# balbasty/torch-interpol

Measured on AMD Instinct MI355X. Metric: Mvox/s grid_pull & grid_push, 256^3 fp32 cubic/dct2, higher is better.
Workload: dtype f32

## Files before the change

### include/interpol_hip.h

```cpp
#ifndef INTERPOL_HIP_H
#define INTERPOL_HIP_H

#include <stdint.h>

#ifdef __cplusplus
extern "C" {
#endif

#define INTERPOL_ABI_VERSION 1

enum {
    INTERPOL_F32  = 0,
    INTERPOL_F64  = 1,
    INTERPOL_BF16 = 2,
    INTERPOL_F16  = 3
};

enum {
    INTERPOL_OK          =  0,
    INTERPOL_E_DIM       = -1,
    INTERPOL_E_ORDER     = -2,
    INTERPOL_E_BOUND     = -3,
    INTERPOL_E_DTYPE     = -4,
    INTERPOL_E_SHAPE     = -5,
    INTERPOL_E_NULL      = -6,
    INTERPOL_E_EXTRAP    = -7,
    INTERPOL_E_PREFILTER = -8,
    INTERPOL_E_SCRATCH   = -9,
    INTERPOL_E_STRIDE    = -10,
    INTERPOL_E_LAUNCH    = -11
};

typedef struct interpol_problem {
    int32_t abi_version;
    int32_t dim;
    int32_t dtype;
    int32_t grid_dtype;
    int32_t extrapolate;
    int32_t bound[3];
    int32_t order[3];
    int32_t flags;
    int64_t batch;
    int64_t channels;
    int64_t vol_shape[3];
    int64_t grid_shape[3];
    int64_t vol_stride[5];
    int64_t grid_stride[5];
    int64_t val_stride[7];
} interpol_problem;

#define INTERPOL_FLAG_NO_FASTPATH   1
#define INTERPOL_FLAG_ACCUMULATE    2
#define INTERPOL_FLAG_FORCE_TILED   4
#define INTERPOL_FLAG_SEPARABLE_GRID 8
#define INTERPOL_FLAG_DISPLACEMENT  16
#define INTERPOL_FLAG_WITH_COUNT    32
#define INTERPOL_FLAG_BINNED_SCATTER 64
#define INTERPOL_FLAG_AUTO_SCATTER  (1 << 24)
#define INTERPOL_FLAG_SMALL_TILES (1 << 25)
#define INTERPOL_FLAG_SERIAL_ITEMS (1 << 26)
#define INTERPOL_FLAG_GENERAL_KERNELS (1 << 27)
#define INTERPOL_FLAG_AFFINE_GRID   128

int64_t interpol_scatter_workspace(const interpol_problem *p, int32_t count_only);
int interpol_pull(const interpol_problem *p, const void *vol, const void *grid, void *val, void *stream);
int64_t interpol_pull_workspace(const interpol_problem *p);
int interpol_pull_ws(const interpol_problem *p, const void *vol, const void *grid, void *val, void *workspace, int64_t workspace_bytes, void *stream);
int interpol_grad_ws(const interpol_problem *p, const void *vol, const void *grid, void *val, void *workspace, int64_t workspace_bytes, void *stream);
int interpol_push(const interpol_problem *p, const void *val, const void *grid, void *vol,
                  void *scratch, int64_t scratch_bytes, void *stream);
int interpol_count(const interpol_problem *p, const void *grid, void *vol,
                   void *scratch, int64_t scratch_bytes, void *stream);
int interpol_grad(const interpol_problem *p, const void *vol, const void *grid, void *val, void *stream);
int interpol_pushgrad(const interpol_problem *p, const void *val, const void *grid, void *vol,
                      void *scratch, int64_t scratch_bytes, void *stream);
int interpol_hess(const interpol_problem *p, const void *vol, const void *grid, void *val, void *stream);

int interpol_pull_backward(const interpol_problem *p, const void *grad_out, const void *vol, const void *grid,
                           void *grad_vol, void *grad_grid, void *scratch, int64_t scratch_bytes, void *stream);
int interpol_push_backward(const interpol_problem *p, const void *grad_vol_out, const void *val, const void *grid,
                           void *grad_val, void *grad_grid, void *stream);
int interpol_count_backward(const interpol_problem *p, const void *grad_vol_out, const void *grid,
                            void *grad_grid, void *stream);
int interpol_push_backward_ws(const interpol_problem *p, const void *grad_vol_out, const void *val, const void *grid,
                              void *grad_val, void *grad_grid, void *workspace, int64_t workspace_bytes, void *stream);

int64_t interpol_affine_backward_workspace(const interpol_problem *p);
int interpol_pull_backward_affine(const interpol_problem *p, const void *grad_out, const void *vol,
                                  const void *mat, void *grad_mat,
                                  void *workspace, int64_t workspace_bytes, void *stream);
int interpol_push_backward_affine(const interpol_problem *p, const void *grad_vol_out,
                                  const void *val , const void *mat, void *grad_mat,
                                  void *workspace, int64_t workspace_bytes, void *stream);

int interpol_compose(const interpol_problem *p, const void *left, const void *right, void *out, void *stream);
int interpol_compose_backward_right(const interpol_problem *p, const void *grad_out, const void *left, const void *right,
                                    void *grad_right, void *stream);

int64_t interpol_push_bricks_workspace(const interpol_problem *p);
int interpol_push_bricks(const interpol_problem *p, const void *val, const void *grid, void *vol,
                         void *workspace, int64_t workspace_bytes, void *stream);

int interpol_pull_labels(const interpol_problem *p, const void *vol, const void *grid, void *val, void *stream);

int interpol_resample_1d(int32_t dtype, int32_t lin_dtype, int32_t order, int32_t bound, int32_t extrapolate, int32_t mode,
                         int32_t adjoint, int64_t outer, int64_t n_samples, int64_t n_lattice, int64_t inner,
                         const void *src, const void *lin, void *dst, void *stream);
int32_t interpol_resample_1d_gathers(int32_t dtype, int64_t n_samples, int64_t inner);

int interpol_spline_filter(void *data, int32_t dtype, int64_t outer, int64_t n, int64_t inner,
                           int32_t bound, int32_t order, void *stream);
int interpol_spline_filter_to(const void *src, void *data, int32_t dtype, int64_t outer, int64_t n, int64_t inner,
                              int32_t bound, int32_t order, void *stream);

// ... 21 lines not shown
```

### torch-interpol_amd/csrc/push_owner.hip

```cpp
#include "sorted_util.hpp"

namespace ip {
namespace owner {

using namespace sorted;

constexpr int BR = 16;
constexpr int OFF = 160;
constexpr int BOX = BR + 3;
constexpr int PZ = BOX;
constexpr int PLANE = BOX * PZ;
constexpr int BOXSLOTS = BOX * PLANE;
constexpr int NCELL = BR * BR * BR;
constexpr int CAPD = 128;
constexpr int CAPX = 512;
constexpr int NT = 512;
constexpr int NS = TS * TS * TS;
constexpr int NT1 = 512, VPT1 = NS / NT1;
constexpr int LB = 6, NBIN = LB * LB * LB;
constexpr int HDR_SHELL = 34;
constexpr int KMIX = 13;
template <int K> constexpr int KSV = K == KMIX ? 3 : K;
template <int K> __device__ __forceinline__ int kd(const KParams &p, int d) { return K == KMIX ? p.order[d] : K; }
#ifdef IP_OWNER_MIX_TU
#define IP_KS KSV<K>
#define IP_KD(d) kd<K>(p, d)
#define IP_WX(i) own_weight_x<K>(p, tx, i)
#define IP_MU magic_units_p<K>(p)
#else
#define IP_KS K
#define IP_KD(d) K
#define IP_WX(i) weight_x<K>(tx, i)
#define IP_MU magic_units<K>()
#endif

constexpr int NLO = OFF / BR, NHI = (OFF + 3 + BR - 1) / BR;
struct BrickGrid {
    int nb[3];
    int lo[3], top[3], nin[3], split[3];
    int per_item;
    int item;
    int capd;
};
__host__ __device__ __forceinline__ bool folds(int bound, int n) { return (bound == B_REPLICATE || bound == B_DCT1 || bound == B_DCT2) && n >= 2 * BR; }
static BrickGrid brick_grid(const KParams &k)
{
    BrickGrid g;
    const bool mixed = k.order[0] != k.order[1] || k.order[0] != k.order[2];
    for (int d = 0; d < 3; ++d) {
        const int K = mixed ? 3 : k.order[d], n = k.vol_n[d];
        const bool f = folds(k.bound[d], n);
        g.lo[d] = f ? -(BOX - 1) / 2 : 0;
        g.top[d] = f ? n - (BOX + 1) / 2 + BR : (n - K > 0 ? n - K : 0);
        g.nin[d] = (g.top[d] - g.lo[d] + BR - 1) / BR;
        if (f) {
            const int c = g.top[d] - g.lo[d] - BR * (g.nin[d] - 1);
            if (c < K) { g.top[d] -= c; g.nin[d] -= 1; }
        }
        g.split[d] = f ? g.nin[d] / 2 : (g.nin[d] > 0 ? g.nin[d] - 1 : 0);
        g.nb[d] = NLO + g.nin[d] + NHI;
    }
    g.per_item = g.nb[0] * g.nb[1] * g.nb[2];
    g.item = g.per_item; g.capd = 128;
    return g;
}
__host__ __device__ __forceinline__ int brick_and_cell(int ft, int lo, int top, int nin, int split)
{
    if (ft < lo) return ((ft - lo + OFF) >> 4) | (((ft - lo + OFF) & (BR - 1)) << 16);
    if (ft >= top) return (NLO + nin + ((ft - top) >> 4)) | (((ft - top) & (BR - 1)) << 16);
    const int u = ft - lo, v = top - 1 - ft;
    const bool hi = u >= BR * split && (v >> 4) < nin - 1 - split;
    return hi ? (NLO + nin - 1 - (v >> 4)) | ((BR - 1 - (v & (BR - 1))) << 16) : (NLO + (u >> 4)) | ((u & (BR - 1)) << 16);
}
__host__ __device__ __forceinline__ int brick_origin(int bk, int lo, int top, int nin, int split)
{
    if (bk < NLO) return lo + bk * BR - OFF;
    if (bk >= NLO + nin) return top + (bk - NLO - nin) * BR;
    const int j = bk - NLO;
    return j <= split ? lo + j * BR : top - (nin - j) * BR;
}

struct BinSmem {
    int lo[3], total;
    int cnt[NBIN];
    int base[NBIN];
    int bmx[2];
    int orph, pad_;
    int gbk[NBIN];
};

template <typename T>
__device__ __forceinline__ float src_value(const KParams &p, const T *__restrict__ val, int64_t b, int64_t o, int ch, float m)
{
    if (val == nullptr || ch >= p.C) return m;
    return m * Cvt<float, T>::ld(val[b * p.val_sb + ch * p.val_sc + o]);
}

template <typename T, int K, int GM>
__device__ __forceinline__ void scatter_direct(const KParams &p, const T *__restrict__ val, const float *__restrict__ grid, float *__restrict__ vol,
                                            int64_t b, TileGeom g, int tid, unsigned mask, int nch)
{
    Lattice L;
#pragma unroll
    for (int d = 0; d < 3; ++d) { L.bound[d] = p.bound[d]; L.n[d] = p.vol_n[d]; L.ss[d] = p.vol_ss[d] / 4; L.k[d] = kd<K>(p, d); }
    L.lin = 0;
#pragma unroll 1
    for (int v = 0; v < VPT1; ++v) {
        if (!((mask >> v) & 1)) continue;
        int ox, oy, oz; float x[3];
        sample_pos(g, tid + NT1 * v, ox, oy, oz);
        load_xyz<GM>(p, grid, b, g, ox, oy, oz, x);
        const int64_t o = ((int64_t)ox * g.gy + oy) * g.gz + oz;
        const float m = inb_mask(p, x);
        if (KSV<K> == 1 && p.mode == MODE_ISO0) {
            const long long pk0 = wrap_outofline(L.bound[0], __float2int_rn(rintf(x[0])), L.n[0]);
            const long long pk1 = wrap_outofline(L.bound[1], __float2int_rn(rintf(x[1])), L.n[1]);
            const long long pk2 = wrap_outofline(L.bound[2], __float2int_rn(rintf(x[2])), L.n[2]);
            const float sgn = (float)((int)(pk0 >> 32) * (int)(pk1 >> 32) * (int)(pk2 >> 32));
            float *q = vol + b * p.vol_sb + (int)(pk0 & 0xffffffffll) * L.ss[0] + (int)(pk1 & 0xffffffffll) * L.ss[1] + (int)(pk2 & 0xffffffffll) * L.ss[2];
#pragma unroll 1
            for (int ch = 0; ch < nch; ++ch)
                __hip_atomic_fetch_add(q + (int64_t)ch * p.vol_sc, src_value<T>(p, val, b, o, ch, m) * sgn, __ATOMIC_RELAXED, __HIP_MEMORY_SCOPE_AGENT);
            continue;
        }
        int ii[3]; float tt[3];
#pragma unroll
        for (int d = 0; d < 3; ++d) split(kd<K>(p, d), x[d], ii[d], tt[d]);
#pragma unroll 1
        for (int ch = 0; ch < nch; ++ch)
            tiled::scatter_one_thread(L, vol + b * p.vol_sb + ch * p.vol_sc, src_value<T>(p, val, b, o, ch, m), ii[0], ii[1], ii[2], tt[0], tt[1], tt[2]);
    }
}

template <typename T, int K, int GM>
__device__ __forceinline__ void gather_direct(const KParams &p, const T *__restrict__ img, const float *__restrict__ grid, T *__restrict__ out,
                                              int64_t b, TileGeom g, int tid, unsigned mask)
{
    Lattice L;
#pragma unroll
    for (int d = 0; d < 3; ++d) { L.bound[d] = p.bound[d]; L.n[d] = p.vol_n[d]; L.ss[d] = p.vol_ss[d] / (int)sizeof(T); L.k[d] = kd<K>(p, d); }
    L.lin = 0;
#pragma unroll 1
    for (int v = 0; v < VPT1; ++v) {
        if (!((mask >> v) & 1)) continue;
        int ox, oy, oz; float x[3];
        sample_pos(g, tid + NT1 * v, ox, oy, oz);
        load_xyz<GM>(p, grid, b, g, ox, oy, oz, x);
        const int64_t o = ((int64_t)ox * g.gy + oy) * g.gz + oz;
        const float m = inb_mask(p, x);
        int ii[3]; float tt[3];
#pragma unroll
        for (int d = 0; d < 3; ++d) split(kd<K>(p, d), x[d], ii[d], tt[d]);
#pragma unroll 1
        for (int ch = 0; ch < p.C; ++ch)
            out[b * p.val_sb + ch * p.val_sc + o] = Cvt<float, T>::st(m * tiled::gather_one_thread<T>(L, img + b * p.vol_sb + ch * p.vol_sc, ii[0], ii[1], ii[2], tt[0], tt[1], tt[2], -1));
    }
}

template <typename T, int K, int GM>
__device__ __forceinline__ void gradc_direct(const KParams &p, const T *__restrict__ img, const T *__restrict__ gout, const float *__restrict__ grid,
                                             float *__restrict__ ggrid, int64_t b, TileGeom g, int tid, unsigned mask)
{
    Lattice L;
#pragma unroll
    for (int d = 0; d < 3; ++d) { L.bound[d] = p.bound[d]; L.n[d] = p.vol_n[d]; L.ss[d] = p.vol_ss[d] / (int)sizeof(T); L.k[d] = kd<K>(p, d); }
    L.lin = 0;
#pragma unroll 1
    for (int v = 0; v < VPT1; ++v) {
        if (!((mask >> v) & 1)) continue;
        int ox, oy, oz; float x[3];
        sample_pos(g, tid + NT1 * v, ox, oy, oz);
        load_xyz<GM>(p, grid, b, g, ox, oy, oz, x);
        const int64_t o = ((int64_t)ox * g.gy + oy) * g.gz + oz;
        const float m = inb_mask(p, x);
        int ii[3]; float tt[3];
#pragma unroll
        for (int d = 0; d < 3; ++d) split(kd<K>(p, d), x[d], ii[d], tt[d]);
        float a[3] = { 0.f, 0.f, 0.f };
#pragma unroll 1
        for (int ch = 0; ch < p.C; ++ch) {
            const float gv = gout ? Cvt<float, T>::ld(gout[b * p.val_sb + ch * p.val_sc + o]) : 1.f;
#pragma unroll 1
            for (int d = 0; d < 3; ++d)
                a[d] = __builtin_fmaf(gv, tiled::gather_one_thread<T>(L, img + b * p.vol_sb + ch * p.vol_sc, ii[0], ii[1], ii[2], tt[0], tt[1], tt[2], d), a[d]);
        }
        float *dst = ggrid + (b * p.N + o) * 3;
        dst[0] = a[0] * m; dst[1] = a[1] * m; dst[2] = a[2] * m;
    }
}

template <typename T, int K, int GM>
__device__ __forceinline__ void grad_direct(const KParams &p, const T *__restrict__ img, const float *__restrict__ grid, T *__restrict__ out,
                                            int64_t b, TileGeom g, int tid, unsigned mask)
{
    Lattice L;
#pragma unroll
    for (int d = 0; d < 3; ++d) { L.bound[d] = p.bound[d]; L.n[d] = p.vol_n[d]; L.ss[d] = p.vol_ss[d] / (int)sizeof(T); L.k[d] = kd<K>(p, d); }
    L.lin = 0;
#pragma unroll 1
    for (int v = 0; v < VPT1; ++v) {
        if (!((mask >> v) & 1)) continue;
        int ox, oy, oz; float x[3];
        sample_pos(g, tid + NT1 * v, ox, oy, oz);
        load_xyz<GM>(p, grid, b, g, ox, oy, oz, x);
        const int64_t o = ((int64_t)ox * g.gy + oy) * g.gz + oz;
        const float m = inb_mask(p, x);
        int ii[3]; float tt[3];
#pragma unroll
        for (int d = 0; d < 3; ++d) split(kd<K>(p, d), x[d], ii[d], tt[d]);
#pragma unroll 1
        for (int ch = 0; ch < p.C; ++ch)
#pragma unroll 1
            for (int d = 0; d < 3; ++d)
                out[b * p.val_sb + ch * p.val_sc + 3 * o + d] =
                    Cvt<float, T>::st(m * tiled::gather_one_thread<T>(L, img + b * p.vol_sb + ch * p.vol_sc, ii[0], ii[1], ii[2], tt[0], tt[1], tt[2], d));
    }
}

template <typename T, int K, int GM, int IDX = 0>
__global__ __launch_bounds__(NT1, 4) void own_bin(KParams p, BrickGrid bg, const T *__restrict__ val, const float *__restrict__ grid,
                                               float *__restrict__ vol, int *__restrict__ ndesc, uint2 *__restrict__ desc,
                                               float4 *__restrict__ rec, float *__restrict__ vals, unsigned short *__restrict__ meta,
                                               int *__restrict__ bmax, int64_t nrec,
                                               int gx, int gy, int gz, int nty, int ntz, int ntiles, const int *__restrict__ gate,
                                               const T *__restrict__ aux, const int *__restrict__ all, int blk0)
{
    const int blk = (int)blockIdx.x + blk0;
    if (IDX) { const bool every = all && *all == 1; if (gate ? (gate[blk] == 0 && !every) : (all && !every)) return; }
    else if (gate && *gate != 1) return;
    extern __shared__ __attribute__((aligned(16))) unsigned char smem_raw[];
    BinSmem &sm = *reinterpret_cast<BinSmem *>(smem_raw);
    const int tid = threadIdx.x;
    const int64_t b = blk / ntiles;
    const TileGeom g = tile_geom(blk % ntiles, gx, gy, gz, nty, ntz);
    const int nch = (IDX || val == nullptr) ? 1 : p.C + p.cc;
    for (int i = tid; i < NBIN; i += NT1) { sm.cnt[i] = 0; sm.gbk[i] = -1; }
    if (tid < 2) sm.bmx[tid] = 0;
    if (tid == 2) sm.orph = 0;
    if (tid < 3) sm.lo[tid] = 0x7fffffff;
    float c[VPT1][3], v0[VPT1], v1[VPT1];
    unsigned valid = 0;
    prof_mark(-1);
    const bool has0 = !IDX && val != nullptr && p.C > 0, has1 = !IDX && val != nullptr && p.C > 1;
    const T *vp0 = has0 ? val + b * p.val_sb : reinterpret_cast<const T *>(grid);
    const T *vp1 = has1 ? val + b * p.val_sb + p.val_sc : reinterpret_cast<const T *>(grid);
#pragma unroll
    for (int v = 0; v < VPT1; ++v) {
        int ox, oy, oz;
        sample_pos(g, tid + NT1 * v, ox, oy, oz);
        if (ox < gx && oy < gy && oz < gz) valid |= 1u << v;
        ox = ox < gx ? ox : gx - 1; oy = oy < gy ? oy : gy - 1; oz = oz < gz ? oz : gz - 1;
        load_xyz<GM>(p, grid, b, g, ox, oy, oz, c[v]);
        const int64_t o = ((int64_t)ox * gy + oy) * gz + oz;
        if (IDX) { v0[v] = __int_as_float((int)o); v1[v] = 0.f; continue; }
        v0[v] = Cvt<float, T>::ld(vp0[has0 ? o : 0]);
        v1[v] = Cvt<float, T>::ld(vp1[has1 ? o : 0]);
    }
    unsigned inbits = 0;
#pragma unroll
    for (int v = 0; v < VPT1 && !IDX; ++v) {
        const float m = inb_mask(p, c[v]);
        v0[v] = has0 ? v0[v] * m : m; v1[v] = has1 ? v1[v] * m : m;
        if (KSV<K> == 1 && m != 0.f) inbits |= 1u << v;
    }
    if (KSV<K> == 1 && !IDX && p.mode == MODE_ISO0) {
#pragma unroll
        for (int v = 0; v < VPT1; ++v) { c[v][0] = rintf(c[v][0]); c[v][1] = rintf(c[v][1]); c[v][2] = rintf(c[v][2]); }
    }
    int bx[VPT1][3];
    unsigned ok = 0;
    int mn[3] = { 0x7fffffff, 0x7fffffff, 0x7fffffff };
#pragma unroll
    for (int v = 0; v < VPT1; ++v) {
        bool in = (valid >> v) & 1;
#pragma unroll
        for (int d = 0; d < 3; ++d) {
            const float fl = floorf(c[v][d] - 0.5f * (float)(kd<K>(p, d) - 1));
            in = in && fl >= (float)(bg.lo[d] - OFF) && fl < (float)(bg.top[d] + NHI * BR);
            bx[v][d] = in ? brick_and_cell(__float2int_rz(fl), bg.lo[d], bg.top[d], bg.nin[d], bg.split[d]) : 0;
        }
        if (in) {
            ok |= 1u << v;
#pragma unroll
            for (int d = 0; d < 3; ++d) mn[d] = (bx[v][d] & 0xffff) < mn[d] ? (bx[v][d] & 0xffff) : mn[d];
        }
    }
    __syncthreads();
    prof_mark(0);
#pragma unroll
    for (int d = 0; d < 3; ++d) {
        const int a = wave_min(mn[d]);
        if ((tid & 63) == 0) atomicMin(&sm.lo[d], a);
    }
    __syncthreads();
    const int lo[3] = { sm.lo[0], sm.lo[1], sm.lo[2] };
    int lbin[VPT1];
    unsigned local = 0;
#pragma unroll
    for (int v = 0; v < VPT1; ++v) {
        const int r0 = (bx[v][0] & 0xffff) - lo[0], r1 = (bx[v][1] & 0xffff) - lo[1], r2 = (bx[v][2] & 0xffff) - lo[2];
        const bool l = ((ok >> v) & 1) && (unsigned)r0 < (unsigned)LB && (unsigned)r1 < (unsigned)LB && (unsigned)r2 < (unsigned)LB;
        lbin[v] = l ? ((r0 * LB + r1) * LB + r2) | ((bx[v][0] >> 16) << 16 | (bx[v][1] >> 16) << 12 | (bx[v][2] >> 16) << 8) : 0;
        if (l) { local |= 1u << v; lbin[v] |= atomicAdd(&sm.cnt[lbin[v] & 255], 1) << 20; }
    }
    __syncthreads();
    prof_mark(1);
    const int64_t tilebase = (int64_t)blk * NS;
    constexpr int PER = (NBIN + 63) / 64;
    int slot[PER];
    if (tid < 64) {
        int cn[PER], s = 0;
#pragma unroll
        for (int i = 0; i < PER; ++i) { const int e = tid * PER + i; cn[i] = e < NBIN ? sm.cnt[e] : 0; s += cn[i]; }
        int incl = s;
#pragma unroll
        for (int o = 1; o < 64; o <<= 1) { const int t = __shfl_up(incl, o); if (tid >= o) incl += t; }
        int run = incl - s;
        if (tid == 63) sm.total = incl;
#pragma unroll
        for (int i = 0; i < PER; ++i) {
            const int e = tid * PER + i;
            const int r0 = e / (LB * LB), r1 = (e / LB) % LB, r2 = e % LB;
            const int bk = (int)b * bg.item + ((lo[0] + r0) * bg.nb[1] + (lo[1] + r1)) * bg.nb[2] + (lo[2] + r2);
            slot[i] = 0;
            if (e < NBIN) sm.base[e] = run;
            if (e < NBIN && cn[i] > 0) slot[i] = atomicAdd(&ndesc[bk], 1);
            run += cn[i];
        }
    }
    __syncthreads();
    prof_mark(2);
    int pos[VPT1];
#pragma unroll
    for (int v = 0; v < VPT1; ++v)
        pos[v] = ((local >> v) & 1) ? (sm.base[lbin[v] & 255] + (int)((unsigned)lbin[v] >> 20)) | (((lbin[v] >> 8) & 0xfff) << 16) : -1;
    const bool two = nch > 1;
    int amx0 = 0, amx1 = 0;
#pragma unroll
    for (int v = 0; v < VPT1; ++v) {
        if (pos[v] < 0) continue;
        const int64_t at = tilebase + (pos[v] & 0xffff);
        rec[at] = make_float4(c[v][0], c[v][1], c[v][2], v0[v]);
        if (IDX) continue;
        meta[at] = (unsigned short)(pos[v] >> 16);
        const int a0 = __float_as_int(__builtin_fabsf(v0[v]));
        amx0 = a0 > amx0 ? a0 : amx0;
        if (two) {
            vals[at] = v1[v];
            const int a1 = __float_as_int(__builtin_fabsf(v1[v]));
            amx1 = a1 > amx1 ? a1 : amx1;
        }
    }
    for (int ch = 2; ch < nch && !IDX; ++ch) {
#pragma unroll
        for (int v = 0; v < VPT1; ++v) {
            if (pos[v] < 0) continue;
            int ox, oy, oz;
            sample_pos(g, tid + NT1 * v, ox, oy, oz);
            vals[(int64_t)(ch - 1) * nrec + tilebase + (pos[v] & 0xffff)] = src_value<T>(p, val, b, ((int64_t)ox * gy + oy) * gz + oz, ch, KSV<K> == 1 ? (float)((inbits >> v) & 1u) : inb_mask(p, c[v]));
        }
    }
    if (tid < 64) {
#pragma unroll
        for (int i = 0; i < PER; ++i) {
            const int e = tid * PER + i;
            const int cn = e < NBIN ? sm.cnt[e] : 0;
            if (cn <= 0) continue;
            const int r0 = e / (LB * LB), r1 = (e / LB) % LB, r2 = e % LB;
            const int bk = (int)b * bg.item + ((lo[0] + r0) * bg.nb[1] + (lo[1] + r1)) * bg.nb[2] + (lo[2] + r2);
            if (slot[i] < bg.capd) {
                desc[(int64_t)bk * bg.capd + slot[i]] = make_uint2((unsigned)(tilebase + sm.base[e]), (unsigned)cn);
                sm.gbk[e] = bk;
                const int bc[3] = { lo[0] + r0, lo[1] + r1, lo[2] + r2 };
                bool shell = false;
#pragma unroll
                for (int d = 0; d < 3; ++d) shell = shell || bc[d] < NLO + (p.bound[d] == B_DST1 ? 1 : 0) || bc[d] >= NLO + bg.nin[d];
                if (!IDX && shell) ndesc[HDR_SHELL - 64] = 1;
                if (IDX && slot[i] == 0) bmax[1 + atomicAdd(&bmax[0], 1)] = bk;
            } else { sm.cnt[e] = -1; sm.orph = 1; }
        }
    }
    if (!IDX) {
        amx0 = wave_max(amx0); amx1 = wave_max(amx1);
        if ((tid & 63) == 0) { if (amx0) atomicMax(&sm.bmx[0], amx0); if (amx1) atomicMax(&sm.bmx[1], amx1); }
    }
    __syncthreads();
    for (int e = tid; e < NBIN && !IDX; e += NT1) {
        const int bk = sm.gbk[e];
        if (bk < 0) continue;
        if (sm.bmx[0]) atomicMax(&bmax[2 * (int64_t)bk], sm.bmx[0]);
        if (sm.bmx[1]) atomicMax(&bmax[2 * (int64_t)bk + 1], sm.bmx[1]);
    }
    unsigned direct = valid & ~local;
    if (sm.orph) {
#pragma unroll
        for (int v = 0; v < VPT1; ++v)
            if (((local >> v) & 1) && sm.cnt[lbin[v] & 255] < 0) direct |= 1u << v;
    }
    if (IDX == 3) { if (direct) grad_direct<T, K, GM>(p, val, grid, reinterpret_cast<T *>(vol), b, g, tid, direct); return; }
    if (IDX == 2) { if (direct) gradc_direct<T, K, GM>(p, val, aux, grid, vol, b, g, tid, direct); return; }
    if (IDX) { if (direct) gather_direct<T, K, GM>(p, val, grid, reinterpret_cast<T *>(vol), b, g, tid, direct); return; }
    if (direct) scatter_direct<T, K, GM>(p, val, grid, vol, b, g, tid, direct, nch);
}

constexpr int VPT = 12;
constexpr int NPIECE = VPT * (NT / 64);
constexpr int BATCH = NPIECE * 64;
constexpr int NCLS = 16;
constexpr int NHW = NT / NCLS;
constexpr unsigned PMASK = 0x1ffffffu;
static_assert(NPIECE <= 128, "a queue entry is piece << 6 | lane in 16 bits");

struct AccSmem {
    int   taboff[3][BOX + 1];
    float tabsgn[3][BOX + 1];
    unsigned ppref[CAPX];
    unsigned start[CAPX];
    uint2 piece[NPIECE];
    int   cmax[2];
    int   dmax, n, npieces;
    int   rlo[3], rhi[3];
    int   qcnt[NCLS];
    int   qsur[NCLS + 1], qhol[NCLS + 1];
    int   qeff[NCLS], qcap;
    union alignas(16) {
        struct {
            unsigned cells[NCELL / 2];
            unsigned short queue[BATCH];
        };
        unsigned nreg[BOX * BOX * (BOX + 1) / 2];
    };
    unsigned long long box[BOXSLOTS];
};
constexpr int NZ = BOX + 1;
static_assert(sizeof(AccSmem) <= 80 * 1024, "two workgroups per CU");
static_assert(sizeof(unsigned) * (BOX * BOX * NZ / 2) <= sizeof(unsigned) * (NCELL / 2) + sizeof(unsigned short) * BATCH, "the stencil counts fit in cells + queue");

constexpr float MAGIC = 12582912.f;
constexpr unsigned MAGIC_ODD = 301u;
template <int K> __device__ __forceinline__ float magic_units() { return K == 3 ? 4194304.f * 0.999f * 3.375f : (K == 2 ? 4194304.f * 0.999f * (64.f / 27.f) : 4194304.f * 0.999f); }
template <int K> __device__ __forceinline__ float magic_cbmax() { return 2147483648.f * 0.99f / magic_units<K>(); }
template <int K> __device__ __forceinline__ float magic_units_p(const KParams &p)
{
    if (K != KMIX) return magic_units<K>();
    float u = 4194304.f * 0.999f;
#pragma unroll
    for (int d = 0; d < 3; ++d) u *= p.order[d] == 3 ? 1.5f : (p.order[d] == 2 ? 4.f / 3.f : 1.f);
    return u;
}

// ... 1137 lines not shown
        if (cnt[2] == NS) { atomicAdd(&hdr->nbox, boxvol); atomicAdd(&hdr->nfull, 1); atomicAdd(&hdr->ncorner, cornervol); }
        __threadfence();
        if (atomicAdd(&hdr->done, 1) == (int)gridDim.x - 1) {
            const int ns = atomicAdd(&hdr->nslow, 0), nf = atomicAdd(&hdr->nfar, 0), nn = atomicAdd(&hdr->nvalid, 0);
            const int nb = atomicAdd(&hdr->nbox, 0), nt = atomicAdd(&hdr->nfull, 0), nc = atomicAdd(&hdr->ncorner, 0);
            const bool rough = nch > 1 && (int64_t)nb > (int64_t)BOXVOL * nt && (int64_t)nb * 10 > (int64_t)nc * 16;
            const bool dense = (int64_t)nc <= (int64_t)DENSEVOL * nt;
            if (nch == -2) hdr->gate = ((int64_t)ns * 1000 > (int64_t)nn * PULLOUT && (int64_t)nf * 64 <= nn) ? 1 : 0;
            else if (nch < 0) hdr->gate = (((int64_t)ns * 250 > nn || dense) && (int64_t)nf * 64 <= nn) ? 1 : 0;
            else hdr->gate = (((int64_t)ns * 250 > nn || rough) && (int64_t)nf * 64 <= nn) ? 1 : 0;
        }
    }
}

struct Workspace {
    int *flags;
    ProbeHdr *hdr; int *ndesc; int *bmax; uint2 *desc; float4 *rec; float *vals; unsigned short *meta;
    int64_t nrec; int nbricks;
};
static int64_t align256(int64_t x) { return (x + 255) & ~(int64_t)255; }

static int64_t layout(const KParams &k, int B, int ntiles, int nch, void *base, Workspace *w, int64_t nflags = 0, bool shared = false)
{
    const BrickGrid bg = brick_grid(k);
    const int64_t nbricks = (int64_t)bg.per_item * (shared ? 1 : B);
    const int64_t nrec = (int64_t)ntiles * NS * B;
    int64_t o = 0;
    unsigned char *p = (unsigned char *)base;
    const int64_t o_hdr = o; o += 256;
    const int64_t o_nd = o; o += nbricks * 4;
    const int64_t o_bm = o; o += nbricks * 8;
    const int64_t o_fl = o; o += nflags * 4; o = align256(o);
    const int64_t o_desc = o; o += align256(nbricks * (shared ? CAPX : CAPD) * 8);
    const int64_t o_rec = o; o += align256(nrec * 16);
    const int64_t o_val = o; o += align256(nrec * 4 * (nch > 1 ? nch - 1 : 0));
    const int64_t o_meta = o; o += align256(nrec * 2);
    if (w) {
        w->hdr = (ProbeHdr *)(p + o_hdr); w->ndesc = (int *)(p + o_nd); w->desc = (uint2 *)(p + o_desc);
        w->rec = (float4 *)(p + o_rec); w->vals = (float *)(p + o_val); w->meta = (unsigned short *)(p + o_meta);
        w->bmax = (int *)(p + o_bm); w->flags = (int *)(p + o_fl);
        w->nrec = nrec; w->nbricks = (int)nbricks;
    }
    return o;
}

static int tile_count(const interpol_problem *p)
{
    int64_t n = 1;
    for (int d = 0; d < 3; ++d) n *= (p->grid_shape[d] + TS - 1) / TS;
    return n > 0x7fffffff ? 0 : (int)n;
}

int mix_launch_bin(int dtype, int idx, const KParams &k, const BrickGrid &bg, const Workspace &w, const void *val, const void *grid, void *vol,
                   const int *gate, const void *aux, const int *all, int gx, int gy, int gz, int ntiles, int b0, int nb, hipStream_t st);
int mix_launch_acc(const KParams &k, const BrickGrid &bg, const Workspace &w, void *vol, int nch, int color, int b0, int nb, const int *gate,
                   int *ctr, unsigned nblocks, hipStream_t st);
int mix_launch_gather(int grad, const KParams &k, const BrickGrid &bg, const Workspace &w, const void *vol, void *val, const int *gate,
                      const void *gout, unsigned nblocks, hipStream_t st);

#ifdef IP_OWNER_MIX_TU
int mix_launch_bin(int dtype, int idx, const KParams &k, const BrickGrid &bg, const Workspace &w, const void *val, const void *grid, void *vol,
                   const int *gate, const void *aux, const int *all, int gx, int gy, int gz, int ntiles, int b0, int nb, hipStream_t st)
{
    const int nty = (gy + TS - 1) / TS, ntz = (gz + TS - 1) / TS;
    const dim3 tgrid((unsigned)(ntiles * nb));
#define IP_MIX_BIN(T, IDX)                                                                                              \
    {                                                                                                                   \
        const int attr = big_lds<own_bin<T, KMIX, 0, IDX>>(sizeof(BinSmem));                                            \
        if (attr) return attr;                                                                                          \
        hipLaunchKernelGGL((own_bin<T, KMIX, 0, IDX>), tgrid, dim3(NT1), sizeof(BinSmem), st, k, bg, (const T *)val, (const float *)grid, \
                           (float *)vol, w.ndesc, w.desc, w.rec, w.vals, w.meta, w.bmax, w.nrec, gx, gy, gz, nty, ntz, ntiles, gate, (const T *)aux, all, ntiles * b0); \
    }
    if (idx == 0) { if (dtype == INTERPOL_F32) IP_MIX_BIN(float, 0) else if (dtype == INTERPOL_BF16) IP_MIX_BIN(bf16_t, 0) else if (dtype == INTERPOL_F16) IP_MIX_BIN(f16_t, 0) else return INTERPOL_E_DTYPE; }
    else if (idx == 1) IP_MIX_BIN(float, 1) else if (idx == 2) IP_MIX_BIN(float, 2) else IP_MIX_BIN(float, 3)
#undef IP_MIX_BIN
    const hipError_t e = hipGetLastError();
    return e == hipSuccess ? 0 : (int)e;
}
int mix_launch_acc(const KParams &k, const BrickGrid &bg, const Workspace &w, void *vol, int nch, int color, int b0, int nb, const int *gate,
                   int *ctr, unsigned nblocks, hipStream_t st)
{
    const int attr = big_lds<own_accumulate<KMIX>>(sizeof(AccSmem));
    if (attr) return attr;
    hipLaunchKernelGGL((own_accumulate<KMIX>), dim3(nblocks), dim3(NT), sizeof(AccSmem), st, k, bg, (const int *)w.ndesc,
                       (const uint2 *)w.desc, (const float4 *)w.rec, (const float *)w.vals, (const unsigned short *)w.meta,
                       (const int *)w.bmax, w.nrec, (float *)vol, nch, color, nb, gate, ctr, b0, (const int *)w.hdr + HDR_SHELL);
    const hipError_t e = hipGetLastError();
    return e == hipSuccess ? 0 : (int)e;
}
int mix_launch_gather(int grad, const KParams &k, const BrickGrid &bg, const Workspace &w, const void *vol, void *val, const int *gate,
                      const void *gout, unsigned nblocks, hipStream_t st)
{
#define IP_MIX_GAT(GR)                                                                                                  \
    {                                                                                                                   \
        const int attr = big_lds<own_gather<KMIX, GR>>(sizeof(GatSmem));                                                \
        if (attr) return attr;                                                                                          \
        hipLaunchKernelGGL((own_gather<KMIX, GR>), dim3(nblocks), dim3(NT), sizeof(GatSmem), st, k, bg, (const int *)w.ndesc, (const uint2 *)w.desc, \
                           (const float4 *)w.rec, (const int *)w.bmax, (int *)w.hdr + 40, (const float *)vol, (float *)val, gate, (const float *)gout); \
    }
    if (grad == 1) IP_MIX_GAT(1) else if (grad == 2) IP_MIX_GAT(2) else IP_MIX_GAT(0)
#undef IP_MIX_GAT
    const hipError_t e = hipGetLastError();
    return e == hipSuccess ? 0 : (int)e;
}
#endif

}

#ifndef IP_OWNER_MIX_TU

static bool shared_target(const interpol_problem *p) { return p->vol_stride[0] == 0 && p->batch > 1; }
static bool mixed_orders(const KParams &k) { return k.order[0] != k.order[1] || k.order[0] != k.order[2]; }
static bool owner_eligible(const interpol_problem *p, const KParams &k, bool scatter = false)
{
    const bool shared = scatter && shared_target(p);
    if (p->dim != 3 || p->batch > 4096) return false;
    if (!(p->flags & (INTERPOL_FLAG_BINNED_SCATTER | INTERPOL_FLAG_AUTO_SCATTER))) return false;
    if (k.order[0] != k.order[1] || k.order[0] != k.order[2]) {
        for (int d = 0; d < 3; ++d) if (k.order[d] < 1 || k.order[d] > 3) return false;
        if (k.sep != 0) return false;
    } else if (k.order[0] < (scatter ? 1 : 2) || k.order[0] > 3) return false;
    int64_t n = 1, nv = 1, nb = shared ? 1 : p->batch;
    for (int d = 0; d < 3; ++d) {
        n *= p->grid_shape[d]; nv *= p->vol_shape[d];
        nb *= owner::NLO + owner::NHI + (p->vol_shape[d] + 15 + owner::BR - 1) / owner::BR;
        if (p->grid_shape[d] > 0x7fffffff / 4) return false;
    }
    const int64_t nt = owner::tile_count(p);
    if (n < 4096 || nt == 0 || nt * owner::NS * p->batch > 0x7fffffffll || nb > 0x7fffffffll / (shared ? owner::CAPX : owner::CAPD)) return false;
    if ((uint64_t)n * 12ull > 0xffffffffull) return false;
    return (shared ? 8 * n * p->batch : 4 * n) >= nv;
}

int linear_pull_probe(const interpol_problem *p, const KParams &k, const void *grid, void *workspace, hipStream_t st, const int **gate_out, int thr16);
constexpr int NEAREST_THR16 = 24;
static bool nearest_scatter(const KParams &k) { return k.dim == 3 && k.mode == MODE_ISO0 && k.order[0] == 0 && k.order[1] == 0 && k.order[2] == 0; }
static KParams nearest_as_trilinear(const KParams &k)
{
    KParams q = k;
    if (nearest_scatter(k)) { q.order[0] = 1; q.order[1] = 1; q.order[2] = 1; }
    return q;
}

int64_t owner_workspace_bytes(const interpol_problem *p, const KParams &k_in, bool count_only)
{
    const KParams k = nearest_as_trilinear(k_in);
    if (!owner_eligible(p, k, true)) return 0;
    const int nch = count_only ? 1 : k.C + (k.cc ? 1 : 0);
    return owner::layout(k, (int)p->batch, owner::tile_count(p), nch, nullptr, nullptr, 0, shared_target(p));
}

namespace owner {
template <typename T, int IDX = 0>
static int launch_bin(const interpol_problem *p, const KParams &k, const BrickGrid &bg, const Workspace &w, const void *val, const void *grid,
                      void *vol, const int *gate, hipStream_t st, const void *aux = nullptr, const int *all = nullptr,
                      int b0 = 0, int nb = -1)
{
    if (nb < 0) nb = (int)p->batch;
    const int gx = (int)p->grid_shape[0], gy = (int)p->grid_shape[1], gz = (int)p->grid_shape[2];
    const int nty = (gy + TS - 1) / TS, ntz = (gz + TS - 1) / TS;
    const int ntiles = tile_count(p);
    const dim3 tgrid((unsigned)(ntiles * nb));
    if (k.order[0] != k.order[1] || k.order[0] != k.order[2])
        return mix_launch_bin(std::is_same<T, float>::value ? INTERPOL_F32 : (std::is_same<T, bf16_t>::value ? INTERPOL_BF16 : INTERPOL_F16), IDX, k, bg, w,
                              val, grid, vol, gate, aux, all, gx, gy, gz, ntiles, b0, nb, st);
#define IP_OWN_BIN(KK, GM)                                                                                              \
    {                                                                                                                   \
        const int attr = big_lds<own_bin<T, KK, GM, IDX>>(sizeof(BinSmem));                                               \
        if (attr) return attr;                                                                                          \
        hipLaunchKernelGGL((own_bin<T, KK, GM, IDX>), tgrid, dim3(NT1), sizeof(BinSmem), st, k, bg, (const T *)val, (const float *)grid, \
                           (float *)vol, w.ndesc, w.desc, w.rec, w.vals, w.meta, w.bmax, w.nrec, gx, gy, gz, nty, ntz, ntiles, gate, (const T *)aux, all, ntiles * b0); \
    }
#define IP_OWN_BY_GM(KK)                                                                                                \
    { if (k.sep == 0) IP_OWN_BIN(KK, 0) else if (k.sep == 1) IP_OWN_BIN(KK, 1) else if (k.sep == 2) IP_OWN_BIN(KK, 2) else IP_OWN_BIN(KK, 3) }
    if (k.order[0] == 3) IP_OWN_BY_GM(3) else if (k.order[0] == 2) IP_OWN_BY_GM(2) else IP_OWN_BY_GM(1)
#undef IP_OWN_BY_GM
#undef IP_OWN_BIN
    return 0;
}
}

static int chain_counter(int chain, int color)
{
    static const int base[CHAIN_SIDE + 1] = { 16, 8 };
    return color < 8 ? base[chain] + color : 24;
}

int try_owner_push(const interpol_problem *p, const KParams &k_in, const void *val, const void *grid, void *vol,
                   void *workspace, int64_t workspace_bytes, hipStream_t st, const int **gate_out, PendingZero *zf)
{
    using namespace owner;
    const bool nearest = nearest_scatter(k_in);
    const KParams k = nearest_as_trilinear(k_in);
    if (!workspace || !owner_eligible(p, k, true)) return 0;
    const bool count_only = val == nullptr;
    const int nch = count_only ? 1 : k.C + (k.cc ? 1 : 0);
    const int dtype = count_only ? INTERPOL_F32 : p->dtype;
    if (dtype != INTERPOL_F32 && dtype != INTERPOL_BF16 && dtype != INTERPOL_F16) return 0;
    Workspace w;
    if (((uintptr_t)workspace & 255u) != 0) return 0;
    const bool shared = shared_target(p);
    if (layout(k, (int)p->batch, tile_count(p), nch, workspace, &w, 0, shared) > workspace_bytes) return 0;
    BrickGrid bg = brick_grid(k);
    if (shared) { bg.item = 0; bg.capd = CAPX; }
    const bool gated = !(p->flags & INTERPOL_FLAG_BINNED_SCATTER);
    if (nearest && gated && k.sep != 0 && k.sep != 2) return 0;
    const int B = (int)p->batch;
    ChainSet *cs = nullptr;
    if (!shared && B >= 2 && !(p->flags & INTERPOL_FLAG_SERIAL_ITEMS)) {
        hipStreamCaptureStatus cap = hipStreamCaptureStatusNone;
        if (hipStreamIsCapturing(st, &cap) != hipSuccess) { (void)hipGetLastError(); cap = hipStreamCaptureStatusActive; }
        if (cap == hipStreamCaptureStatusNone) cs = chains_acquire();
    }
    bool zero_pending = zf && zf->pending;
    const size_t slice = (size_t)k.vol_sb * 4;
    if (zero_pending && !(cs && zf->ptr == vol && slice * (size_t)B == zf->bytes)) {
        const hipError_t ez = zero_async(zf->ptr, zf->bytes, st);
        if (ez != hipSuccess) { chains_release(cs); return (int)ez; }
        zf->pending = zero_pending = false;
    }
    hipLaunchKernelGGL(own_zero, dim3((unsigned)((64 + 3ll * w.nbricks + 1023) / 1024)), dim3(1024), 0, st, (int *)w.hdr, 64 + 3 * w.nbricks);
    hipError_t e = hipGetLastError();
    if (e != hipSuccess) { chains_release(cs); return (int)e; }
    const int *gate = nullptr;
    if (gated && nearest) {
        const int rp = linear_pull_probe(p, k, grid, w.hdr, st, &gate, NEAREST_THR16);
        if (rp) { chains_release(cs); return rp; }
    } else if (gated) {
        const int gx = (int)p->grid_shape[0], gy = (int)p->grid_shape[1], gz = (int)p->grid_shape[2];
        const int nty = (gy + TS - 1) / TS, ntz = (gz + TS - 1) / TS, ntiles = tile_count(p);
        const long long total = (long long)ntiles * B;
        const dim3 pgrid((unsigned)(total < NPROBE ? total : NPROBE));
#define IP_OWN_PROBE(KK, GM) hipLaunchKernelGGL((own_probe<KK, GM>), pgrid, dim3(NT1), 0, st, k, bg, (const float *)grid, w.hdr, gx, gy, gz, nty, ntz, ntiles, B, nch);
#define IP_OWN_PROBE_GM(KK) { if (k.sep == 0) IP_OWN_PROBE(KK, 0) else if (k.sep == 1) IP_OWN_PROBE(KK, 1) else if (k.sep == 2) IP_OWN_PROBE(KK, 2) else IP_OWN_PROBE(KK, 3) }
        if (k.order[0] == 3 || mixed_orders(k)) IP_OWN_PROBE_GM(3) else if (k.order[0] == 2) IP_OWN_PROBE_GM(2) else IP_OWN_PROBE_GM(1)
#undef IP_OWN_PROBE_GM
#undef IP_OWN_PROBE
        gate = &w.hdr->gate;
    }
    const int nchain = B < CHAIN_SIDE + 1 ? B : CHAIN_SIDE + 1;
    if (cs) {
        bool ok = hipEventRecord(cs->fork, st) == hipSuccess;
        for (int i = 0; i + 1 < nchain && ok; ++i) ok = hipStreamWaitEvent(cs->side[i], cs->fork, 0) == hipSuccess;
        if (!ok) { (void)hipGetLastError(); chains_release(cs); cs = nullptr; }
    }
    if (zero_pending && !cs) {
        const hipError_t ez = zero_async(zf->ptr, zf->bytes, st);
        if (ez != hipSuccess) return (int)ez;
        zf->pending = zero_pending = false;
    }
    const long long want = 2ll * cu_count();
    const bool general = (p->flags & INTERPOL_FLAG_GENERAL_KERNELS) != 0;
    auto enqueue = [&](hipStream_t s, int chain, int b0, int nb) -> int {
        if (zero_pending) {
            const hipError_t ez = zero_async((char *)vol + (size_t)b0 * slice, (size_t)nb * slice, s);
            if (ez != hipSuccess) return (int)ez;
        }
        const int nbin = shared ? B : nb;
        int rc;
        switch (dtype) {
        case INTERPOL_F32: rc = launch_bin<float>(p, k, bg, w, val, grid, vol, gate, s, nullptr, nullptr, b0, nbin); break;
        case INTERPOL_BF16: rc = launch_bin<bf16_t>(p, k, bg, w, val, grid, vol, gate, s, nullptr, nullptr, b0, nbin); break;
        default: rc = launch_bin<f16_t>(p, k, bg, w, val, grid, vol, gate, s, nullptr, nullptr, b0, nbin); break;
        }
        if (rc) return rc;
        for (int color = 0; color < 9; ++color) {
            long long nwork = nb;
            for (int d = 0; d < 3; ++d) nwork *= color_count(color, d, bg);
            if (nwork <= 0) continue;
            const dim3 agrid((unsigned)(nwork < want ? nwork : want));
            int *ctr = (int *)w.hdr + chain_counter(chain, color);
#define IP_OWN_ACC_SH(KK, SH)                                                                                           \
            {                                                                                                           \
                const int attr = big_lds<own_accumulate<KK, false, SH>>(sizeof(AccSmem));                               \
                if (attr) return attr;                                                                                  \
                hipLaunchKernelGGL((own_accumulate<KK, false, SH>), agrid, dim3(NT), sizeof(AccSmem), s, k, bg, (const int *)w.ndesc, \
                                   (const uint2 *)w.desc, (const float4 *)w.rec, (const float *)w.vals, (const unsigned short *)w.meta,  \
                                   (const int *)w.bmax, w.nrec, (float *)vol, nch, color, nb, gate, ctr, b0,           \
                                   (const int *)w.hdr + HDR_SHELL);                                                     \
            }
#define IP_OWN_ACC(KK) { if (color < 8 && !general) IP_OWN_ACC_SH(KK, false) else IP_OWN_ACC_SH(KK, true) }
            if (mixed_orders(k)) { const int rm = mix_launch_acc(k, bg, w, vol, nch, color, b0, nb, gate, ctr, agrid.x, s); if (rm) return rm; }
            else if (k.order[0] == 3) IP_OWN_ACC(3) else if (k.order[0] == 2) IP_OWN_ACC(2)
            else if (nearest) {
                const int attr = big_lds<own_accumulate<1, true>>(sizeof(AccSmem));
                if (attr) return attr;
                hipLaunchKernelGGL((own_accumulate<1, true>), agrid, dim3(NT), sizeof(AccSmem), s, k, bg, (const int *)w.ndesc,
                                   (const uint2 *)w.desc, (const float4 *)w.rec, (const float *)w.vals, (const unsigned short *)w.meta,
                                   (const int *)w.bmax, w.nrec, (float *)vol, nch, color, nb, gate, ctr, b0, (const int *)w.hdr + HDR_SHELL);
            }
            else IP_OWN_ACC(1)
#undef IP_OWN_ACC
#undef IP_OWN_ACC_SH
        }
        const hipError_t el = hipGetLastError();
        return el == hipSuccess ? 0 : (int)el;
    };
    int rc = 0;
    if (!cs) rc = enqueue(st, 0, 0, shared ? 1 : B);
    else {
        for (int c = 1; c <= nchain && rc == 0; ++c) {
            const int ch = c % nchain, b0 = (int)((long long)ch * B / nchain), b1 = (int)((long long)(ch + 1) * B / nchain);
            rc = enqueue(ch ? cs->side[ch - 1] : st, ch, b0, b1 - b0);
        }
        if (zero_pending && rc == 0) zf->pending = false;
        for (int i = 0; i + 1 < nchain; ++i) {
            if (hipEventRecord(cs->join[i], cs->side[i]) == hipSuccess && hipStreamWaitEvent(st, cs->join[i], 0) == hipSuccess) continue;
            (void)hipGetLastError();
            const hipError_t es = hipStreamSynchronize(cs->side[i]);
            if (es != hipSuccess && rc == 0) rc = (int)es;
        }
        chains_release(cs);
    }
    if (rc) return rc;
    if (gate_out) *gate_out = gate;
    return gated ? 2 : 1;
// ... 171 lines not shown
```

### torch-interpol_amd/interpol/_hip.py

```python
import ctypes
import threading
import os

import torch

from .sepgrid import SeparableGrid, AffineGrid, LazyGrid

_PKG_ROOT = os.path.dirname(os.path.dirname(os.path.abspath(__file__)))
LIB_PATH = os.environ.get("INTERPOL_HIP_LIB") or os.path.join(_PKG_ROOT, "lib", "libinterpol_hip.so")

ABI_VERSION = 1
F32, F64, BF16, F16 = 0, 1, 2, 3
FLAG_NO_FASTPATH = 1
FLAG_ACCUMULATE = 2
FLAG_FORCE_TILED = 4
FLAG_SEPARABLE_GRID = 8
FLAG_DISPLACEMENT = 16
FLAG_WITH_COUNT = 32
FLAG_BINNED_SCATTER = 64
FLAG_AUTO_SCATTER = 1 << 24
_ROUTED_2D = (torch.float32, torch.bfloat16, torch.float16)
FLAG_SMALL_TILES = 1 << 25
FLAG_SERIAL_ITEMS = 1 << 26
FLAG_GENERAL_KERNELS = 1 << 27
_POISON_SCRATCH = os.environ.get("INTERPOL_POISON_SCRATCH", "0") not in ("", "0")
_WS_NOCACHE = os.environ.get("INTERPOL_WS_NOCACHE", "0") not in ("", "0")
FLAG_AFFINE_GRID = 128

def _empty(*size, **kw):
    return torch.empty(*size, **kw)


def _scratch(t):
    if _POISON_SCRATCH and t is not None:
        t.view(torch.uint8).fill_(0xff)
    return t


_DTYPE_CODE = {torch.float32: F32, torch.float64: F64, torch.bfloat16: BF16, torch.float16: F16}

SYMBOLS = (
    "interpol_pull", "interpol_push", "interpol_count", "interpol_grad", "interpol_pushgrad",
    "interpol_hess", "interpol_pull_backward", "interpol_push_backward", "interpol_count_backward",
    "interpol_spline_filter", "interpol_spline_filter_to", "interpol_resample_1d", "interpol_resample_1d_gathers", "interpol_pull_labels",
    "interpol_push_bricks", "interpol_push_bricks_workspace", "interpol_host_bound_index", "interpol_host_bound_sign",
    "interpol_host_weight", "interpol_host_weight_f32", "interpol_abi_version",
    "interpol_error_string", "interpol_kernel_name", "interpol_scatter_workspace",
    "interpol_set_handback", "interpol_release_stream", "interpol_has_experiments", "interpol_pull_workspace", "interpol_pull_ws", "interpol_push_backward_ws", "interpol_grad_ws",
    "interpol_affine_backward_workspace", "interpol_pull_backward_affine", "interpol_push_backward_affine",
    "interpol_compose", "interpol_compose_backward_right",
)


class Problem(ctypes.Structure):
    _fields_ = [
        ("abi_version", ctypes.c_int32),
        ("dim", ctypes.c_int32),
        ("dtype", ctypes.c_int32),
        ("grid_dtype", ctypes.c_int32),
        ("extrapolate", ctypes.c_int32),
        ("bound", ctypes.c_int32 * 3),
        ("order", ctypes.c_int32 * 3),
        ("flags", ctypes.c_int32),
        ("batch", ctypes.c_int64),
        ("channels", ctypes.c_int64),
        ("vol_shape", ctypes.c_int64 * 3),
        ("grid_shape", ctypes.c_int64 * 3),
        ("vol_stride", ctypes.c_int64 * 5),
        ("grid_stride", ctypes.c_int64 * 5),
        ("val_stride", ctypes.c_int64 * 7),
    ]


_lib = None


class HipExtensionMissing(ImportError):
# ... 843 lines not shown
```

Measured before the change: 33090.

## Scatter thin shell-brick runs directly with atomics instead of binning

In the push binning kernel, bins that fall on boundary shell bricks and hold only a few samples (at or below a threshold, 16 by default) skip descriptor allocation. They are marked as orphans and scattered straight into the volume with global atomics. Orphaned samples in the non-index path now also go through a new atomic scatter helper instead of the direct path. The goal is to shrink the shell-accumulation work and descriptor traffic for sparse boundary bins, at the cost of extra atomic contention. A new flag disables this, and debug bits choose the threshold.

```diff
diff --git a/include/interpol_hip.h b/include/interpol_hip.h
--- a/include/interpol_hip.h
+++ b/include/interpol_hip.h
@@ -60,6 +60,7 @@
 #define INTERPOL_FLAG_SMALL_TILES (1 << 25)
 #define INTERPOL_FLAG_SERIAL_ITEMS (1 << 26)
 #define INTERPOL_FLAG_GENERAL_KERNELS (1 << 27)
+#define INTERPOL_FLAG_SHELL_RUNS (1 << 28)
 #define INTERPOL_FLAG_AFFINE_GRID   128
 
 int64_t interpol_scatter_workspace(const interpol_problem *p, int32_t count_only);
diff --git a/torch-interpol_amd/csrc/push_owner.hip b/torch-interpol_amd/csrc/push_owner.hip
--- a/torch-interpol_amd/csrc/push_owner.hip
+++ b/torch-interpol_amd/csrc/push_owner.hip
@@ -19,6 +19,7 @@
 constexpr int NT1 = 512, VPT1 = NS / NT1;
 constexpr int LB = 6, NBIN = LB * LB * LB;
 constexpr int HDR_SHELL = 34;
+constexpr int THIN_SHELL_RUN = 16;
 constexpr int KMIX = 13;
 template <int K> constexpr int KSV = K == KMIX ? 3 : K;
 template <int K> __device__ __forceinline__ int kd(const KParams &p, int d) { return K == KMIX ? p.order[d] : K; }
@@ -80,6 +81,15 @@
     return j <= split ? lo + j * BR : top - (nin - j) * BR;
 }
 
+__device__ __forceinline__ bool shell_brick(const KParams &p, const BrickGrid &bg, int b0, int b1, int b2)
+{
+    const int bc[3] = { b0, b1, b2 };
+    bool shell = false;
+#pragma unroll
+    for (int d = 0; d < 3; ++d) shell = shell || bc[d] < NLO + (p.bound[d] == B_DST1 ? 1 : 0) || bc[d] >= NLO + bg.nin[d];
+    return shell;
+}
+
 struct BinSmem {
     int lo[3], total;
     int cnt[NBIN];
@@ -133,6 +143,37 @@
 }
 
 template <typename T, int K, int GM>
+__device__ __forceinline__ void scatter_orphans(const KParams &p, const T *__restrict__ val, const float *__restrict__ grid, float *__restrict__ vol,
+                                             int64_t b, TileGeom g, int tid, unsigned mask, int nch)
+{
+    Lattice L;
+#pragma unroll
+    for (int d = 0; d < 3; ++d) { L.bound[d] = p.bound[d]; L.n[d] = p.vol_n[d]; L.ss[d] = p.vol_ss[d] / 4; L.k[d] = kd<K>(p, d); }
+    L.lin = 0;
+#pragma unroll 1
+    for (int v = 0; v < VPT1; ++v) {
+        unsigned long long todo = __ballot((mask >> v) & 1);
+#pragma unroll 1
+        while (todo) {
+            const int lane = __ffsll((long long)todo) - 1;
+            todo &= todo - 1;
+            int ox, oy, oz; float x[3];
+            sample_pos(g, (tid & ~63) + lane + NT1 * v, ox, oy, oz);
+            load_xyz<GM>(p, grid, b, g, ox, oy, oz, x);
+            const int64_t o = ((int64_t)ox * g.gy + oy) * g.gz + oz;
+            const float m = inb_mask(p, x);
+            if (KSV<K> == 1 && p.mode == MODE_ISO0) { x[0] = rintf(x[0]); x[1] = rintf(x[1]); x[2] = rintf(x[2]); }
+            int off;
+            const float w = tiled::tap_weight_t<-1, -1>(L, x[0], x[1], x[2], tid & 63, &off, nullptr);
+            float *q = vol + b * p.vol_sb + off;
+#pragma unroll 1
+            for (int ch = 0; ch < nch && w != 0.f; ++ch)
+                __hip_atomic_fetch_add(q + (int64_t)ch * p.vol_sc, src_value<T>(p, val, b, o, ch, m) * w, __ATOMIC_RELAXED, __HIP_MEMORY_SCOPE_AGENT);
+        }
+    }
+}
+
+template <typename T, int K, int GM>
 __device__ __forceinline__ void gather_direct(const KParams &p, const T *__restrict__ img, const float *__restrict__ grid, T *__restrict__ out,
                                               int64_t b, TileGeom g, int tid, unsigned mask)
 {
@@ -223,7 +264,7 @@
                                                float4 *__restrict__ rec, float *__restrict__ vals, unsigned short *__restrict__ meta,
                                                int *__restrict__ bmax, int64_t nrec,
                                                int gx, int gy, int gz, int nty, int ntz, int ntiles, const int *__restrict__ gate,
-                                               const T *__restrict__ aux, const int *__restrict__ all, int blk0)
+                                               const T *__restrict__ aux, const int *__restrict__ all, int blk0, int thin)
 {
     const int blk = (int)blockIdx.x + blk0;
     if (IDX) { const bool every = all && *all == 1; if (gate ? (gate[blk] == 0 && !every) : (all && !every)) return; }
@@ -317,6 +358,18 @@
         for (int o = 1; o < 64; o <<= 1) { const int t = __shfl_up(incl, o); if (tid >= o) incl += t; }
         int run = incl - s;
         if (tid == 63) sm.total = incl;
+        unsigned shl = 0;
+        int nsh = 0;
+        if (!IDX && thin != 0) {
+#pragma unroll
+            for (int i = 0; i < PER; ++i) {
+                const int e = tid * PER + i;
+                if (e < NBIN && cn[i] > 0 && shell_brick(p, bg, lo[0] + e / (LB * LB), lo[1] + (e / LB) % LB, lo[2] + e % LB)) { shl |= 1u << i; nsh += cn[i]; }
+            }
+#pragma unroll
+            for (int o = 32; o > 0; o >>= 1) nsh += __shfl_xor(nsh, o);
+        }
+        const int lim = thin < 0 ? -thin : thin;
 #pragma unroll
         for (int i = 0; i < PER; ++i) {
             const int e = tid * PER + i;
@@ -324,7 +377,7 @@
             const int bk = (int)b * bg.item + ((lo[0] + r0) * bg.nb[1] + (lo[1] + r1)) * bg.nb[2] + (lo[2] + r2);
             slot[i] = 0;
             if (e < NBIN) sm.base[e] = run;
-            if (e < NBIN && cn[i] > 0) slot[i] = atomicAdd(&ndesc[bk], 1);
+            if (e < NBIN && cn[i] > 0) slot[i] = (((shl >> i) & 1) && (thin > 0 ? nsh : cn[i]) <= lim) ? 0x7fffffff : atomicAdd(&ndesc[bk], 1);
             run += cn[i];
         }
     }
@@ -371,11 +424,7 @@
             if (slot[i] < bg.capd) {
                 desc[(int64_t)bk * bg.capd + slot[i]] = make_uint2((unsigned)(tilebase + sm.base[e]), (unsigned)cn);
                 sm.gbk[e] = bk;
-                const int bc[3] = { lo[0] + r0, lo[1] + r1, lo[2] + r2 };
-                bool shell = false;
-#pragma unroll
-                for (int d = 0; d < 3; ++d) shell = shell || bc[d] < NLO + (p.bound[d] == B_DST1 ? 1 : 0) || bc[d] >= NLO + bg.nin[d];
-                if (!IDX && shell) ndesc[HDR_SHELL - 64] = 1;
+                if (!IDX && shell_brick(p, bg, lo[0] + r0, lo[1] + r1, lo[2] + r2)) ndesc[HDR_SHELL - 64] = 1;
                 if (IDX && slot[i] == 0) bmax[1 + atomicAdd(&bmax[0], 1)] = bk;
             } else { sm.cnt[e] = -1; sm.orph = 1; }
         }
@@ -393,9 +442,12 @@
     }
     unsigned direct = valid & ~local;
     if (sm.orph) {
+        unsigned orphan = 0;
 #pragma unroll
         for (int v = 0; v < VPT1; ++v)
-            if (((local >> v) & 1) && sm.cnt[lbin[v] & 255] < 0) direct |= 1u << v;
+            if (((local >> v) & 1) && sm.cnt[lbin[v] & 255] < 0) orphan |= 1u << v;
+        if (IDX) direct |= orphan;
+        else scatter_orphans<T, K, GM>(p, val, grid, vol, b, g, tid, orphan, nch);
     }
     if (IDX == 3) { if (direct) grad_direct<T, K, GM>(p, val, grid, reinterpret_cast<T *>(vol), b, g, tid, direct); return; }
     if (IDX == 2) { if (direct) gradc_direct<T, K, GM>(p, val, aux, grid, vol, b, g, tid, direct); return; }
@@ -1639,7 +1691,7 @@
 }
 
 int mix_launch_bin(int dtype, int idx, const KParams &k, const BrickGrid &bg, const Workspace &w, const void *val, const void *grid, void *vol,
-                   const int *gate, const void *aux, const int *all, int gx, int gy, int gz, int ntiles, int b0, int nb, hipStream_t st);
+                   const int *gate, const void *aux, const int *all, int gx, int gy, int gz, int ntiles, int b0, int nb, hipStream_t st, int thin);
 int mix_launch_acc(const KParams &k, const BrickGrid &bg, const Workspace &w, void *vol, int nch, int color, int b0, int nb, const int *gate,
                    int *ctr, unsigned nblocks, hipStream_t st);
 int mix_launch_gather(int grad, const KParams &k, const BrickGrid &bg, const Workspace &w, const void *vol, void *val, const int *gate,
@@ -1647,7 +1699,7 @@
 
 #ifdef IP_OWNER_MIX_TU
 int mix_launch_bin(int dtype, int idx, const KParams &k, const BrickGrid &bg, const Workspace &w, const void *val, const void *grid, void *vol,
-                   const int *gate, const void *aux, const int *all, int gx, int gy, int gz, int ntiles, int b0, int nb, hipStream_t st)
+                   const int *gate, const void *aux, const int *all, int gx, int gy, int gz, int ntiles, int b0, int nb, hipStream_t st, int thin)
 {
     const int nty = (gy + TS - 1) / TS, ntz = (gz + TS - 1) / TS;
     const dim3 tgrid((unsigned)(ntiles * nb));
@@ -1656,7 +1708,7 @@
         const int attr = big_lds<own_bin<T, KMIX, 0, IDX>>(sizeof(BinSmem));                                            \
         if (attr) return attr;                                                                                          \
         hipLaunchKernelGGL((own_bin<T, KMIX, 0, IDX>), tgrid, dim3(NT1), sizeof(BinSmem), st, k, bg, (const T *)val, (const float *)grid, \
-                           (float *)vol, w.ndesc, w.desc, w.rec, w.vals, w.meta, w.bmax, w.nrec, gx, gy, gz, nty, ntz, ntiles, gate, (const T *)aux, all, ntiles * b0); \
+                           (float *)vol, w.ndesc, w.desc, w.rec, w.vals, w.meta, w.bmax, w.nrec, gx, gy, gz, nty, ntz, ntiles, gate, (const T *)aux, all, ntiles * b0, thin); \
     }
     if (idx == 0) { if (dtype == INTERPOL_F32) IP_MIX_BIN(float, 0) else if (dtype == INTERPOL_BF16) IP_MIX_BIN(bf16_t, 0) else if (dtype == INTERPOL_F16) IP_MIX_BIN(f16_t, 0) else return INTERPOL_E_DTYPE; }
     else if (idx == 1) IP_MIX_BIN(float, 1) else if (idx == 2) IP_MIX_BIN(float, 2) else IP_MIX_BIN(float, 3)
@@ -1741,7 +1793,7 @@
 template <typename T, int IDX = 0>
 static int launch_bin(const interpol_problem *p, const KParams &k, const BrickGrid &bg, const Workspace &w, const void *val, const void *grid,
                       void *vol, const int *gate, hipStream_t st, const void *aux = nullptr, const int *all = nullptr,
-                      int b0 = 0, int nb = -1)
+                      int b0 = 0, int nb = -1, int thin = 0)
 {
     if (nb < 0) nb = (int)p->batch;
     const int gx = (int)p->grid_shape[0], gy = (int)p->grid_shape[1], gz = (int)p->grid_shape[2];
@@ -1750,13 +1802,13 @@
     const dim3 tgrid((unsigned)(ntiles * nb));
     if (k.order[0] != k.order[1] || k.order[0] != k.order[2])
         return mix_launch_bin(std::is_same<T, float>::value ? INTERPOL_F32 : (std::is_same<T, bf16_t>::value ? INTERPOL_BF16 : INTERPOL_F16), IDX, k, bg, w,
-                              val, grid, vol, gate, aux, all, gx, gy, gz, ntiles, b0, nb, st);
+                              val, grid, vol, gate, aux, all, gx, gy, gz, ntiles, b0, nb, st, thin);
 #define IP_OWN_BIN(KK, GM)                                                                                              \
     {                                                                                                                   \
         const int attr = big_lds<own_bin<T, KK, GM, IDX>>(sizeof(BinSmem));                                               \
         if (attr) return attr;                                                                                          \
         hipLaunchKernelGGL((own_bin<T, KK, GM, IDX>), tgrid, dim3(NT1), sizeof(BinSmem), st, k, bg, (const T *)val, (const float *)grid, \
-                           (float *)vol, w.ndesc, w.desc, w.rec, w.vals, w.meta, w.bmax, w.nrec, gx, gy, gz, nty, ntz, ntiles, gate, (const T *)aux, all, ntiles * b0); \
+                           (float *)vol, w.ndesc, w.desc, w.rec, w.vals, w.meta, w.bmax, w.nrec, gx, gy, gz, nty, ntz, ntiles, gate, (const T *)aux, all, ntiles * b0, thin); \
     }
 #define IP_OWN_BY_GM(KK)                                                                                                \
     { if (k.sep == 0) IP_OWN_BIN(KK, 0) else if (k.sep == 1) IP_OWN_BIN(KK, 1) else if (k.sep == 2) IP_OWN_BIN(KK, 2) else IP_OWN_BIN(KK, 3) }
@@ -1838,6 +1890,8 @@
     }
     const long long want = 2ll * cu_count();
     const bool general = (p->flags & INTERPOL_FLAG_GENERAL_KERNELS) != 0;
+    static const int thins[4] = { THIN_SHELL_RUN, 4, 64, 16 };
+    const int thin = (p->flags & INTERPOL_FLAG_SHELL_RUNS) ? 0 : ((k.dbg & 256) ? -1 : 1) * thins[(k.dbg >> 6) & 3];
     auto enqueue = [&](hipStream_t s, int chain, int b0, int nb) -> int {
         if (zero_pending) {
             const hipError_t ez = zero_async((char *)vol + (size_t)b0 * slice, (size_t)nb * slice, s);
@@ -1846,9 +1900,9 @@
         const int nbin = shared ? B : nb;
         int rc;
         switch (dtype) {
-        case INTERPOL_F32: rc = launch_bin<float>(p, k, bg, w, val, grid, vol, gate, s, nullptr, nullptr, b0, nbin); break;
-        case INTERPOL_BF16: rc = launch_bin<bf16_t>(p, k, bg, w, val, grid, vol, gate, s, nullptr, nullptr, b0, nbin); break;
-        default: rc = launch_bin<f16_t>(p, k, bg, w, val, grid, vol, gate, s, nullptr, nullptr, b0, nbin); break;
+        case INTERPOL_F32: rc = launch_bin<float>(p, k, bg, w, val, grid, vol, gate, s, nullptr, nullptr, b0, nbin, thin); break;
+        case INTERPOL_BF16: rc = launch_bin<bf16_t>(p, k, bg, w, val, grid, vol, gate, s, nullptr, nullptr, b0, nbin, thin); break;
+        default: rc = launch_bin<f16_t>(p, k, bg, w, val, grid, vol, gate, s, nullptr, nullptr, b0, nbin, thin); break;
         }
         if (rc) return rc;
         for (int color = 0; color < 9; ++color) {
diff --git a/torch-interpol_amd/interpol/_hip.py b/torch-interpol_amd/interpol/_hip.py
--- a/torch-interpol_amd/interpol/_hip.py
+++ b/torch-interpol_amd/interpol/_hip.py
@@ -23,6 +23,7 @@
 FLAG_SMALL_TILES = 1 << 25
 FLAG_SERIAL_ITEMS = 1 << 26
 FLAG_GENERAL_KERNELS = 1 << 27
+FLAG_SHELL_RUNS = 1 << 28
 _POISON_SCRATCH = os.environ.get("INTERPOL_POISON_SCRATCH", "0") not in ("", "0")
 _WS_NOCACHE = os.environ.get("INTERPOL_WS_NOCACHE", "0") not in ("", "0")
 FLAG_AFFINE_GRID = 128
```

After: 33550, median of 6. +1.4%, better.
